# qq456cvb/VoteNet

Measured on AMD Instinct MI355X. Metric: SUN RGB-D 20k-pt scenes/sec (fwd+bwd), higher is better.
Workload: dtype f32

## Files before the change

### votenet_amd/csrc/mlp_wgrad_fast.hip

```cpp
#include "mlp_types.h"

namespace votenet {

constexpr int WF_BR = 16;

typedef short tr_v4s __attribute__((ext_vector_type(4)));
typedef __attribute__((address_space(3))) tr_v4s *tr_lds_ptr;
__device__ __forceinline__ uint4 tr_fragment(unsigned lds_off, unsigned four_rows)
{
    const tr_v4s lo = __builtin_amdgcn_ds_read_tr16_b64_v4i16((tr_lds_ptr)(uintptr_t)lds_off);
    const tr_v4s hi = __builtin_amdgcn_ds_read_tr16_b64_v4i16((tr_lds_ptr)(uintptr_t)(lds_off + four_rows));
    const uint2 a = __builtin_bit_cast(uint2, lo), b = __builtin_bit_cast(uint2, hi);
    return make_uint4(a.x, a.y, b.x, b.y);
}

template <int MODE, int TI, int TJ, int BSRC, bool BF3 = false>
__global__ __launch_bounds__(256) __attribute__((amdgpu_waves_per_eu(2, 3))) void mlp_wgrad_fast_kernel(
    MlpIn in, long rows, int cin, int cout, const float *__restrict__ dz, BnSrc bs, float *__restrict__ dw, long rows_per_block)
{
    if (bs.nh_dev != nullptr) {
        const long lim = (long)bs.nh_dev[0] * kPiece;
        rows = lim < rows ? lim : rows;
    }
    constexpr int BI = 64 * TI, BJ = 64 * TJ;
    constexpr int QA = BI / 4, QB = BJ / 4;
    constexpr int NA = WF_BR * QA / 256, NB = WF_BR * QB / 256;
    constexpr int RA = 256 / QA, RB = 256 / QB;
    __shared__ float As[BF3 ? 1 : 2][BF3 ? 1 : WF_BR][BI + 4];
    __shared__ float Bs[BF3 ? 1 : 2][BF3 ? 1 : WF_BR][BJ + 4];
    constexpr int PA = BI * 2 + 64, PB = BJ * 2 + 64;
    __shared__ __attribute__((aligned(16))) unsigned char A3[BF3 ? 2 * 3 * WF_BR * PA : 16];
    __shared__ __attribute__((aligned(16))) unsigned char B3[BF3 ? 2 * 3 * WF_BR * PB : 16];
    const int tid = threadIdx.x, lane = tid & 63;
    const int wv = __builtin_amdgcn_readfirstlane(tid >> 6);
    const int wi = wv >> 1, wj = wv & 1;
    const int i0 = blockIdx.y * BI, j0 = blockIdx.z * BJ;
    const long r_begin = (long)blockIdx.x * rows_per_block;
    if (r_begin >= rows) return;
    const int nrow = (int)((r_begin + rows_per_block < rows ? r_begin + rows_per_block : rows) - r_begin);
    const int nslab = (nrow + WF_BR - 1) / WF_BR;
    const int a_row = tid / QA, a_q = tid % QA;
    const int b_row = tid / QB, b_q = tid % QB;
    const int ka = i0 + a_q * 4;
    const int nb = j0 + b_q * 4;
    const int xc = (MODE == 0) ? cin : in.c;

    const bool affine = (MODE == 0 || MODE == 2 || MODE == 3) && in.in_scale != nullptr;
    float4 wx0 = make_float4(0.f, 0.f, 0.f, 0.f), wx1 = wx0, wx2 = wx0;
    if (MODE == 3) {
        wx0 = *reinterpret_cast<const float4 *>(in.wx + ka);
        wx1 = *reinterpret_cast<const float4 *>(in.wx + cin + ka);
        wx2 = *reinterpret_cast<const float4 *>(in.wx + 2 * cin + ka);
    }
    float w0r[4][8], b0r[4];
    if (MODE == 2) {
#pragma unroll
        for (int d = 0; d < 8; d++) {
            const float4 w4 = d < in.k0 ? *reinterpret_cast<const float4 *>(in.w0 + (size_t)d * cin + ka) : make_float4(0.f, 0.f, 0.f, 0.f);
            w0r[0][d] = w4.x;
            w0r[1][d] = w4.y;
            w0r[2][d] = w4.z;
            w0r[3][d] = w4.w;
        }
        const float4 b4 = in.b0 ? *reinterpret_cast<const float4 *>(in.b0 + ka) : make_float4(0.f, 0.f, 0.f, 0.f);
        b0r[0] = b4.x;
        b0r[1] = b4.y;
        b0r[2] = b4.z;
        b0r[3] = b4.w;
    }
    float4 csc = make_float4(1.f, 1.f, 1.f, 1.f), csh = make_float4(0.f, 0.f, 0.f, 0.f);
    if (affine) {
        csc = *reinterpret_cast<const float4 *>(in.in_scale + ka);
        csh = *reinterpret_cast<const float4 *>(in.in_shift + ka);
    }
    const float x_floor = (affine && in.in_relu) ? 0.0f : -__builtin_inff();
    float4 kA, kB, kC, kS, kH;
    kA = kB = kC = kS = kH = make_float4(0.f, 0.f, 0.f, 0.f);
    if (BSRC == 1 || BSRC == 2 || BSRC == 4) {
        kA = *reinterpret_cast<const float4 *>(bs.coef + nb);
        kB = *reinterpret_cast<const float4 *>(bs.coef + cout + nb);
        kC = *reinterpret_cast<const float4 *>(bs.coef + 2 * cout + nb);
        kS = *reinterpret_cast<const float4 *>(bs.coef + 3 * cout + nb);
        kH = *reinterpret_cast<const float4 *>(bs.coef + 4 * cout + nb);
    }
    if (BSRC == 3) {
        kS = *reinterpret_cast<const float4 *>(bs.coef + nb);
        kH = *reinterpret_cast<const float4 *>(bs.coef + cout + nb);
    }
    const float b_floor = (BSRC == 3 && bs.relu) ? 0.0f : -__builtin_inff();
    const float *xb = (MODE == 0) ? in.x + (size_t)r_begin * cin + ka : (MODE == 2) ? in.u8 + (size_t)r_begin * 8 : (MODE == 3) ? in.ptab + ka : in.feat + ka;
    const float4 *geob = (MODE == 3) ? reinterpret_cast<const float4 *>(in.geo) + r_begin : nullptr;
    const float *zb = (BSRC == 0 ? dz : bs.z) + (size_t)r_begin * cout + nb;
    const float *gb = (BSRC == 1 || BSRC == 4) ? bs.da + (size_t)r_begin * cout + nb : nullptr;
    const int *idxb = (MODE == 1) ? in.idx + r_begin : nullptr;
    const unsigned grows = (MODE == 1) ? (unsigned)in.m * (unsigned)in.nsample : 1u;

    struct Regs {
        float4 a[NA], b[NB], g[NB];
        float4 a2[(MODE == 2 || MODE == 3) ? NA : 1];
        int4 m[NB];
        float mu[NB];
        int s;
    };
    Regs R[2];
    struct Pix {
        int i;
        float4 g;
    };
    Pix pidx[NA];
    auto clampr = [&](int lr) { return lr < nrow ? lr : nrow - 1; };
    auto load_idx = [&](int s) {
        if (MODE == 1 || MODE == 3) {
#pragma unroll
            for (int h = 0; h < NA; h++) {
                const int lr = clampr(s * WF_BR + a_row + h * RA);
                if (MODE == 1) pidx[h].i = idxb[lr];
                else pidx[h].g = geob[lr];
            }
        }
    };
    auto load_slab = [&](Regs &r, int s, const Pix (&pi)[NA]) {
        r.s = s;
#pragma unroll
        for (int h = 0; h < NA; h++) {
            const int lr = clampr(s * WF_BR + a_row + h * RA);
            if (MODE == 0) {
                r.a[h] = *reinterpret_cast<const float4 *>(xb + (size_t)((unsigned)lr * (unsigned)cin));
            } else if (MODE == 2) {
                r.a[h] = *reinterpret_cast<const float4 *>(xb + (size_t)((unsigned)lr * 8u));
                r.a2[h] = *reinterpret_cast<const float4 *>(xb + (size_t)((unsigned)lr * 8u) + 4);
            } else if (MODE == 3) {
                r.a[h] = *reinterpret_cast<const float4 *>(xb + (size_t)__float_as_uint(pi[h].g.w) * cin);
                r.a2[h] = pi[h].g;
            } else {
                const unsigned scene = (unsigned)(r_begin + lr) / grows;
                r.a[h] = *reinterpret_cast<const float4 *>(xb + ((size_t)scene * in.n + pi[h].i) * xc);
            }
        }
#pragma unroll
        for (int h = 0; h < NB; h++) {
            const int lr = clampr(s * WF_BR + b_row + h * RB);
            const unsigned off = (unsigned)lr * (unsigned)cout;
            r.b[h] = *reinterpret_cast<const float4 *>(zb + (size_t)off);
            if (BSRC == 1 || BSRC == 4) r.g[h] = *reinterpret_cast<const float4 *>(gb + (size_t)off);
            if (BSRC == 4) {
                const unsigned gr = (unsigned)(r_begin + lr);
                r.mu[h] = (gr % (unsigned)kPiece) == 0u ? bs.wh[gr / (unsigned)kPiece] : 1.0f;
            }
            if (BSRC == 2) {
                const unsigned gr = (unsigned)(r_begin + lr);
                const unsigned grp = bs.pool_shift >= 0 ? gr >> bs.pool_shift : gr / (unsigned)bs.pool_k;
                r.g[h] = *reinterpret_cast<const float4 *>(bs.gout + (size_t)grp * cout + nb);
                r.m[h] = *reinterpret_cast<const int4 *>(bs.argmax + (size_t)grp * cout + nb);
            }
        }
    };
    auto store_slab = [&](int buf, const Regs &r) {
#pragma unroll
        for (int h = 0; h < NA; h++) {
            float4 v = r.a[h];
            if (MODE == 2) {
                const float4 v2 = r.a2[h];
                const float uu[8] = {v.x, v.y, v.z, v.w, v2.x, v2.y, v2.z, v2.w};
                const f32x2 z01 = narrow_z2(uu, w0r[0], w0r[1], b0r[0], b0r[1]), z23 = narrow_z2(uu, w0r[2], w0r[3], b0r[2], b0r[3]);
                v.x = z01.x;
                v.y = z01.y;
                v.z = z23.x;
                v.w = z23.y;
            }
            if (MODE == 3) {
                const float4 g = r.a2[h];
                const f32x2 z01 = assembled_z2(v.x, v.y, g, wx0.x, wx0.y, wx1.x, wx1.y, wx2.x, wx2.y);
                const f32x2 z23 = assembled_z2(v.z, v.w, g, wx0.z, wx0.w, wx1.z, wx1.w, wx2.z, wx2.w);
                v.x = z01.x;
                v.y = z01.y;
                v.z = z23.x;
                v.w = z23.y;
            }
            v.x = fmaxf(v.x * csc.x + csh.x, x_floor);
            v.y = fmaxf(v.y * csc.y + csh.y, x_floor);
            v.z = fmaxf(v.z * csc.z + csh.z, x_floor);
            v.w = fmaxf(v.w * csc.w + csh.w, x_floor);
            if constexpr (BF3) {
                unsigned h0, m0, l0, h1, m1, l1;
                split3(v.x, v.y, h0, m0, l0);
                split3(v.z, v.w, h1, m1, l1);
                unsigned char *d = A3 + ((size_t)(buf * 3) * WF_BR + a_row + h * RA) * PA + a_q * 8;
                *reinterpret_cast<uint2 *>(d) = make_uint2(h0, h1);
                *reinterpret_cast<uint2 *>(d + WF_BR * PA) = make_uint2(m0, m1);
                *reinterpret_cast<uint2 *>(d + 2 * WF_BR * PA) = make_uint2(l0, l1);
            } else {
                *reinterpret_cast<float4 *>(&As[buf][a_row + h * RA][a_q * 4]) = v;
            }
// ... 83 lines not shown
    const int nslab2 = (nslab + 1) & ~1;
    for (int s = 0; s < nslab2; s += 2) {
#pragma unroll
        for (int par = 0; par < 2; par++) {
            Regs &rs = R[par ^ 1];
            if constexpr (BF3) {
                const unsigned g = (unsigned)lane >> 4, sl = (unsigned)lane & 15u;
                const unsigned la = ((g >> 1) * 8u + (sl >> 2)) * PA + ((g & 1u) * 16u + (sl & 3u) * 4u) * 2u + (unsigned)(wi * TI) * 64u;
                const unsigned lb = ((g >> 1) * 8u + (sl >> 2)) * PB + ((g & 1u) * 16u + (sl & 3u) * 4u) * 2u + (unsigned)(wj * TJ) * 64u;
                const unsigned a0 = (unsigned)(uintptr_t)A3 + (unsigned)buf * (3u * WF_BR * PA) + la;
                const unsigned b0 = (unsigned)(uintptr_t)B3 + (unsigned)buf * (3u * WF_BR * PB) + lb;
                uint4 fa3[3][TI], fb3[3][TJ];
#pragma unroll
                for (int pc = 0; pc < 3; pc++) {
#pragma unroll
                    for (int t = 0; t < TI; t++) fa3[pc][t] = tr_fragment(a0 + (unsigned)pc * (WF_BR * PA) + (unsigned)t * 64u, 4u * PA);
#pragma unroll
                    for (int t = 0; t < TJ; t++) fb3[pc][t] = tr_fragment(b0 + (unsigned)pc * (WF_BR * PB) + (unsigned)t * 64u, 4u * PB);
                }
                auto mm = [&](int pa, int pb) {
#pragma unroll
                    for (int a = 0; a < TI; a++)
#pragma unroll
                        for (int b = 0; b < TJ; b++)
                            acc[a][b] = __builtin_amdgcn_mfma_f32_32x32x16_bf16(__builtin_bit_cast(bf16x8, fa3[pa][a]),
                                                                                __builtin_bit_cast(bf16x8, fb3[pb][b]), acc[a][b], 0, 0, 0);
                };
#ifdef WG_ABL_HALF
                mm(2, 0);
#else
                mm(2, 0);
                mm(0, 2);
                mm(1, 1);
#endif
                store_slab(buf ^ 1, rs);
#pragma unroll
                for (int h = 0; h < NA; h++) pcur[h] = pidx[h];
                load_idx(s + par + 4);
                load_slab(rs, s + par + 3, pcur);
#ifdef WG_ABL_HALF
                mm(0, 1);
                mm(0, 0);
#else
                mm(1, 0);
                mm(0, 1);
                mm(0, 0);
#endif
                lds_barrier();
                buf ^= 1;
                continue;
            }
            float fa[2][TI], fb[2][TJ];
#pragma unroll
            for (int t = 0; t < TI; t++) fa[0][t] = As[buf][kh][(wi * TI + t) * 32 + l31];
#pragma unroll
            for (int t = 0; t < TJ; t++) fb[0][t] = Bs[buf][kh][(wj * TJ + t) * 32 + l31];
#pragma unroll
            for (int k2 = 0; k2 < WF_BR / 2; k2++) {
                if (k2 == WF_BR / 4) {
                    store_slab(buf ^ 1, rs);
#pragma unroll
                    for (int h = 0; h < NA; h++) pcur[h] = pidx[h];
                    load_idx(s + par + 4);
                    load_slab(rs, s + par + 3, pcur);
                }
                if (k2 + 1 < WF_BR / 2) {
#pragma unroll
                    for (int t = 0; t < TI; t++) fa[(k2 + 1) & 1][t] = As[buf][(k2 + 1) * 2 + kh][(wi * TI + t) * 32 + l31];
#pragma unroll
                    for (int t = 0; t < TJ; t++) fb[(k2 + 1) & 1][t] = Bs[buf][(k2 + 1) * 2 + kh][(wj * TJ + t) * 32 + l31];
                }
                __builtin_amdgcn_sched_barrier(0);
#pragma unroll
                for (int a = 0; a < TI; a++)
#pragma unroll
                    for (int b = 0; b < TJ; b++)
                        acc[a][b] = __builtin_amdgcn_mfma_f32_32x32x2f32(fa[k2 & 1][a], fb[k2 & 1][b], acc[a][b], 0, 0, 0);
                __builtin_amdgcn_sched_barrier(0);
            }
            lds_barrier();
            buf ^= 1;
        }
    }
    const int wrow0 = (MODE == 1) ? 3 : 0;
#pragma unroll
    for (int a = 0; a < TI; a++)
#pragma unroll
        for (int b = 0; b < TJ; b++) {
            const int j = j0 + (wj * TJ + b) * 32 + l31;
#pragma unroll
            for (int e = 0; e < 16; e++) {
                const int i = i0 + (wi * TI + a) * 32 + (e & 3) + 8 * (e >> 2) + 4 * kh;
                const size_t off = (size_t)(wrow0 + i) * cout + j;
                if (bs.part) bs.part[(size_t)blockIdx.x * bs.pstride + off] = acc[a][b][e];
                else unsafeAtomicAdd(&dw[off], acc[a][b][e]);
            }
        }
}

int g_wgrad_fast_wgs = 0;
int g_wgrad_bf3 = 1;
static void plan_fast(long rows, int cin, int cout, int &TIr, int &TJr, int &ti, int &tj, long &rpb, unsigned &gx, bool partials)
{
    TIr = cin % 128 == 0 ? 2 : 1;
    TJr = cout % 128 == 0 ? 2 : 1;
    ti = cin / (64 * TIr);
    tj = cout / (64 * TJr);
    const int wgs = g_wgrad_fast_wgs > 0 ? g_wgrad_fast_wgs : (partials ? 256 : 384);
    long splits = wgs / (ti * tj);
    if (splits < 1) splits = 1;
    rpb = (rows + splits - 1) / splits;
    rpb = (rpb + 2 * WF_BR - 1) / (2 * WF_BR) * (2 * WF_BR);
    if (rpb < 8 * WF_BR) rpb = 8 * WF_BR;
    gx = (unsigned)((rows + rpb - 1) / rpb);
}

long wgrad_fast_slices(long rows, int cin, int cout)
{
    if (cin % 64 != 0 || cout % 64 != 0 || rows <= 0) return 0;
    int TIr, TJr, ti, tj;
    long rpb;
    unsigned gx;
    plan_fast(rows, cin, cout, TIr, TJr, ti, tj, rpb, gx, false);
    return gx;
}

void wgrad_reduce(int nslice, long pstride, long e0, long e1, const float *part, float *dw, hipStream_t st);

template <int MODE, int BSRC>
static bool launch(const MlpIn &d, long rows, int cin, int cout, const float *dz, BnSrc bs, float *dw, hipStream_t st, float *scratch)
{
    int TIr, TJr, ti, tj;
    long rpb;
    unsigned gx;
    plan_fast(rows, cin, cout, TIr, TJr, ti, tj, rpb, gx, scratch != nullptr);
    const int wide = cin > cout ? cin : cout;
    if (rpb * wide >= (1L << 31)) return false;
    const int wrow0 = (MODE == 1) ? 3 : 0;
    bs.part = scratch;
    bs.pstride = (long)(wrow0 + cin) * cout;
    const dim3 grid(gx, ti, tj);
    if (g_wgrad_bf3 && BSRC != 3) {
        if (TIr == 2 && TJr == 2)
            hipLaunchKernelGGL((mlp_wgrad_fast_kernel<MODE, 2, 2, BSRC, true>), grid, dim3(256), 0, st, d, rows, cin, cout, dz, bs, dw, rpb);
        else if (TIr == 2)
            hipLaunchKernelGGL((mlp_wgrad_fast_kernel<MODE, 2, 1, BSRC, true>), grid, dim3(256), 0, st, d, rows, cin, cout, dz, bs, dw, rpb);
        else if (TJr == 2)
            hipLaunchKernelGGL((mlp_wgrad_fast_kernel<MODE, 1, 2, BSRC, true>), grid, dim3(256), 0, st, d, rows, cin, cout, dz, bs, dw, rpb);
        else
            hipLaunchKernelGGL((mlp_wgrad_fast_kernel<MODE, 1, 1, BSRC, true>), grid, dim3(256), 0, st, d, rows, cin, cout, dz, bs, dw, rpb);
    } else if (TIr == 2 && TJr == 2)
        hipLaunchKernelGGL((mlp_wgrad_fast_kernel<MODE, 2, 2, BSRC>), grid, dim3(256), 0, st, d, rows, cin, cout, dz, bs, dw, rpb);
    else if (TIr == 2)
        hipLaunchKernelGGL((mlp_wgrad_fast_kernel<MODE, 2, 1, BSRC>), grid, dim3(256), 0, st, d, rows, cin, cout, dz, bs, dw, rpb);
    else if (TJr == 2)
        hipLaunchKernelGGL((mlp_wgrad_fast_kernel<MODE, 1, 2, BSRC>), grid, dim3(256), 0, st, d, rows, cin, cout, dz, bs, dw, rpb);
    else
        hipLaunchKernelGGL((mlp_wgrad_fast_kernel<MODE, 1, 1, BSRC>), grid, dim3(256), 0, st, d, rows, cin, cout, dz, bs, dw, rpb);
    if (scratch) wgrad_reduce((int)gx, bs.pstride, (long)wrow0 * cout, (long)(wrow0 + cin) * cout, scratch, dw, st);
    return true;
}

bool wgrad_fast_launch(int mode, const MlpIn &d, long rows, int cin, int cout, const float *dz, const BnSrc &bs, int bsrc, float *dw,
                       hipStream_t st, float *scratch)
{
    if (cin % 64 != 0 || cout % 64 != 0 || rows <= 0 || rows >= (1L << 31)) return false;
    auto al = [](const void *p) { return ((uintptr_t)p % 16) == 0; };
    if (!al(dw) || (bsrc == 0 && !al(dz)) || (bsrc != 0 && (!al(bs.z) || !al(bs.coef))) || ((bsrc == 1 || bsrc == 4) && !al(bs.da)) ||
        (bsrc == 2 && (!al(bs.gout) || !al(bs.argmax))))
        return false;
    if (mode == 0) {
        if (!al(d.x) || (d.in_scale && (!al(d.in_scale) || !al(d.in_shift)))) return false;
        if (bsrc == 0) return launch<0, 0>(d, rows, cin, cout, dz, bs, dw, st, scratch);
        if (bsrc == 1) return launch<0, 1>(d, rows, cin, cout, dz, bs, dw, st, scratch);
        if (bsrc == 3) return launch<0, 3>(d, rows, cin, cout, dz, bs, dw, st, scratch);
        return launch<0, 2>(d, rows, cin, cout, dz, bs, dw, st, scratch);
    }
    if (mode == 3) {
        if (!al(d.geo) || !al(d.ptab) || !al(d.wx) || (bsrc != 1 && bsrc != 4)) return false;
        if (d.in_scale && (!al(d.in_scale) || !al(d.in_shift))) return false;
        if (bsrc == 4) return bs.wh != nullptr && rows % 32 == 0 && launch<3, 4>(d, rows, cin, cout, dz, bs, dw, st, scratch);
        return launch<3, 1>(d, rows, cin, cout, dz, bs, dw, st, scratch);
    }
    if (mode == 2) {
        if (!al(d.u8) || !al(d.w0) || (d.b0 && !al(d.b0)) || d.k0 < 1 || d.k0 > 8 || (bsrc != 1 && bsrc != 4)) return false;
        if (d.in_scale && (!al(d.in_scale) || !al(d.in_shift))) return false;
        if (bsrc == 4) return bs.wh != nullptr && rows % 32 == 0 && launch<2, 4>(d, rows, cin, cout, dz, bs, dw, st, scratch);
        return launch<2, 1>(d, rows, cin, cout, dz, bs, dw, st, scratch);
    }
    if (d.c != cin || !al(d.feat) || bsrc != 0) return false;
    return launch<1, 0>(d, rows, cin, cout, dz, bs, dw, st, scratch);
}

}

extern "C" void votenet_debug_wgrad_workgroups(int n) { VN_DEBUG_GATE(); votenet::g_wgrad_fast_wgs = n > 0 ? n : 0; }
extern "C" void votenet_debug_wgrad_bf3(int on) { VN_DEBUG_GATE(); votenet::g_wgrad_bf3 = on ? 1 : 0; }
```

### votenet_amd/csrc/pool_bwd.hip

```cpp
#include "mlp_types.h"
#include <mutex>
#include <set>

namespace votenet {

bool wgrad_fast_launch(int mode, const MlpIn &d, long rows, int cin, int cout, const float *dz, const BnSrc &bs, int bsrc, float *dw,
                       hipStream_t st, float *scratch);
void wgrad_reduce(int nslice, long pstride, long e0, long e1, const float *part, float *dw, hipStream_t st);

static inline int pb_grid(long total, int block, int cap)
{
    long g = (total + block - 1) / block;
    if (g > cap) g = cap;
    return (int)(g < 1 ? 1 : g);
}

__global__ __launch_bounds__(256) void bn_bwd_reduce_zsel_kernel(long groups, int c, const float *__restrict__ gout,
                                                                 const float *__restrict__ zsel, const float *__restrict__ scale,
                                                                 const float *__restrict__ shift, const float *__restrict__ mean,
                                                                 const float *__restrict__ var, float eps, int relu,
                                                                 double *__restrict__ sums, CoefTail tail)
{
    __shared__ float sh1[4][64], sh2[4][64];
    const int cx = threadIdx.x & 63, ry = threadIdx.x >> 6;
// ... 958 lines not shown
                                     below_var, eps, below_relu, below_sums, below_tail, hc, wh, G, stream, nh_dev);
}

static int pool_dgrad_scatter_launch(long groups, int k, int cin, int cout, const float *gout, const int *argmax, const float *zsel,
                                     const float *coef, int relu, const float *wT, float *da, const float *below_z,
                                     const float *below_scale, const float *below_shift, const float *below_mean, const float *below_var,
                                     float eps, int below_relu, double *below_sums, const votenet_coef_tail *below_tail, const int *hc,
                                     const float *wh, int G, void *stream, const int *nh_dev)
{
    hipStream_t st = as_stream(stream);
    const PoolBelow pb = {below_z, below_scale, below_shift, below_mean, below_var, eps, below_relu, below_sums, to_tail(below_tail), g_scatter_reverse, hc, wh, G, nh_dev};
    auto go = [&](auto kern, int ci, int co, int threads = 512) {
        const size_t smem = ((size_t)co * ci + 4 * co + 4 * k) * 4;
        const int per_cu = smem > 80 * 1024 ? 1 : (smem > 40 * 1024 ? 2 : 4);
        static std::set<const void *> raised;
        static std::mutex raised_mu;
        bool fresh;
        {
            std::lock_guard<std::mutex> lock(raised_mu);
            fresh = raised.insert(reinterpret_cast<const void *>(kern)).second;
        }
        if (fresh)
            (void)hipFuncSetAttribute(reinterpret_cast<const void *>(kern), hipFuncAttributeMaxDynamicSharedMemorySize, (int)smem);
        hipLaunchKernelGGL(kern, dim3(pb_grid(groups, 2, 256 * per_cu)), dim3(threads), smem, st, groups, gout, argmax, zsel, coef, relu,
                           wT, da, pb);
    };
    auto gow = [&](auto kern, int ci, int co, int kk, int nwv) {
        const size_t smem = (size_t)co * ci * 4 + (size_t)nwv * ((co + 3 * kk) * 6 + kk * 4);
        const int per_cu = smem > 80 * 1024 ? 1 : (smem > 40 * 1024 ? 2 : 4);
        static std::set<const void *> raised_w;
        static std::mutex raised_w_mu;
        bool fresh;
        {
            std::lock_guard<std::mutex> lock(raised_w_mu);
            fresh = raised_w.insert(reinterpret_cast<const void *>(kern)).second;
        }
        if (fresh)
            (void)hipFuncSetAttribute(reinterpret_cast<const void *>(kern), hipFuncAttributeMaxDynamicSharedMemorySize, (int)smem);
        hipLaunchKernelGGL(kern, dim3(pb_grid(groups, nwv, g_scatter_wgs > 0 ? g_scatter_wgs : 256 * per_cu)), dim3(nwv * 64), smem, st, groups, gout,
                           argmax, zsel, coef, relu, wT, da, pb);
    };
    if (g_scatter_form == 1 || hc) {
#define VN_SCATTER_WAVE(CI, CO, KK, NW)                                                            \
    do {                                                                                           \
        if (below_z) gow(pool_dgrad_scatter_wave_kernel<CI, CO, KK, true, NW>, CI, CO, KK, NW);   \
        else gow(pool_dgrad_scatter_wave_kernel<CI, CO, KK, false, NW>, CI, CO, KK, NW);          \
    } while (0)
        if (hc) {
            if (cin == 64) VN_SCATTER_WAVE(64, 128, kPiece, 8);
            else if (cout == 256) {
                if (g_scatter_nwv == 12) VN_SCATTER_WAVE(128, 256, kPiece, 12);
                else VN_SCATTER_WAVE(128, 256, kPiece, 16);
            }
            else VN_SCATTER_WAVE(128, 128, kPiece, 8);
        } else {
            if (cin == 64) VN_SCATTER_WAVE(64, 128, 64, 8);
            else if (cout == 256) VN_SCATTER_WAVE(128, 256, 64, 8);
            else VN_SCATTER_WAVE(128, 128, 64, 8);
        }
#undef VN_SCATTER_WAVE
        return check_launch("pool_dgrad_scatter");
    }
    if (below_z) {
        if (cin == 128 && cout == 256)
            go(pool_dgrad_scatter_kernel<128, 256, 64, true, 16>, 128, 256, 1024);
        else if (cin == 128)
            go(pool_dgrad_scatter_kernel<128, 128, 64, true>, 128, 128);
        else
            go(pool_dgrad_scatter_kernel<64, 128, 64, true>, 64, 128);
    } else {
        if (cin == 128 && cout == 256)
            go(pool_dgrad_scatter_kernel<128, 256, 64, false, 16>, 128, 256, 1024);
        else if (cin == 128)
            go(pool_dgrad_scatter_kernel<128, 128, 64, false>, 128, 128);
        else
            go(pool_dgrad_scatter_kernel<64, 128, 64, false>, 64, 128);
    }
    return check_launch("pool_dgrad_scatter");
}

#ifndef GRAM_ABL
#define GRAM_ABL 0
#endif
template <int C, int NP = 3>
__global__ __launch_bounds__(256) void gram_bf3_kernel(long rows, const float *__restrict__ x, const float *__restrict__ scale_shift,
                                                       int relu, float *__restrict__ gram, long rows_per_block,
                                                       const float *__restrict__ wh ,
                                                       const int *__restrict__ nh_dev )
{
    if (nh_dev != nullptr) {
        const long lim = (long)nh_dev[0] * kPiece;
        rows = lim < rows ? lim : rows;
    }
    constexpr int KPT = C / 16;
    constexpr int T = C / 64;
    constexpr int PL = C * 4 + 16;
    static_assert(NP == 2 || NP == 3, "pieces per operand");
    constexpr float kA = NP == 2 ? 16.0f : 1.0f, kUn = NP == 2 ? 1.0f / 256.0f : 1.0f;
    __shared__ __attribute__((aligned(16))) unsigned Ts[2][NP][2][PL];
    const int tid = threadIdx.x, lane = tid & 63;
    const int wv = __builtin_amdgcn_readfirstlane(tid >> 6);
    const int wi = wv >> 1, wj = wv & 1;
    const long r_begin = (long)blockIdx.x * rows_per_block;
    if (r_begin >= rows) return;
    const int nrow = (int)((r_begin + rows_per_block < rows ? r_begin + rows_per_block : rows) - r_begin);
    const int nslab = (nrow + 15) / 16;
    const int c = tid % C, rg = tid / C;
    const int kh_w = (C == 128) ? rg : (rg >> 1), d_w = (C == 128) ? 0 : (rg & 1) * 2;
    const float sc = scale_shift[c] * kA, sh = scale_shift[C + c] * kA;
    const float floor_ = relu ? 0.0f : -__builtin_inff();
    const float *xb = x + (size_t)r_begin * C + c;
    float R[2][KPT];
    static_assert(kPiece == 16, "one slab = one piece");
    const bool first_rg = rg == 0;
    const float *whb = wh ? wh + r_begin / kPiece : nullptr;
    const float *whp = whb ? whb : scale_shift;
    float Wq[2] = {1.0f, 1.0f};
    bool abl_prologue = true;
    auto load = [&](float (&r)[KPT], int s, float &wq) {
        if ((GRAM_ABL & 4) && !abl_prologue) return;
#pragma unroll
        for (int i = 0; i < KPT; i++) {
            int lr = s * 16 + rg * KPT + i;
            lr = lr < nrow ? lr : nrow - 1;
            r[i] = xb[(size_t)lr * C];
        }
        const int sw = (whb != nullptr && s * 16 < nrow) ? s : 0;
        wq = whp[sw];
    };
    auto store = [&](int buf, const float (&r)[KPT], int s, float wq) {
        if ((GRAM_ABL & 8) && !abl_prologue) return;
        float v[KPT];
#pragma unroll
        for (int i = 0; i < KPT; i++) {
            v[i] = fmaxf(r[i] * sc + sh, floor_);
            if (s * 16 + rg * KPT + i >= nrow) v[i] = 0.0f;
        }
        if (whb != nullptr && first_rg && s * 16 < nrow) v[0] *= sqrtf(wq);
        if constexpr (NP == 2) {
            unsigned h[KPT / 2], l[KPT / 2];
#pragma unroll
            for (int i = 0; i < KPT / 2; i++) split2(v[2 * i], v[2 * i + 1], h[i], l[i]);
            if constexpr (C == 128) {
                *reinterpret_cast<uint4 *>(&Ts[buf][0][kh_w][c * 4]) = make_uint4(h[0], h[1], h[2], h[3]);
                *reinterpret_cast<uint4 *>(&Ts[buf][1][kh_w][c * 4]) = make_uint4(l[0], l[1], l[2], l[3]);
            } else {
                *reinterpret_cast<uint2 *>(&Ts[buf][0][kh_w][c * 4 + d_w]) = make_uint2(h[0], h[1]);
                *reinterpret_cast<uint2 *>(&Ts[buf][1][kh_w][c * 4 + d_w]) = make_uint2(l[0], l[1]);
            }
            return;
        }
        unsigned h[KPT / 2], m[KPT / 2], l[KPT / 2];
#pragma unroll
        for (int i = 0; i < KPT / 2; i++) split3(v[2 * i], v[2 * i + 1], h[i], m[i], l[i]);
        if constexpr (C == 128) {
            *reinterpret_cast<uint4 *>(&Ts[buf][0][kh_w][c * 4]) = make_uint4(h[0], h[1], h[2], h[3]);
            *reinterpret_cast<uint4 *>(&Ts[buf][1][kh_w][c * 4]) = make_uint4(m[0], m[1], m[2], m[3]);
            *reinterpret_cast<uint4 *>(&Ts[buf][NP - 1][kh_w][c * 4]) = make_uint4(l[0], l[1], l[2], l[3]);
        } else {
            *reinterpret_cast<uint2 *>(&Ts[buf][0][kh_w][c * 4 + d_w]) = make_uint2(h[0], h[1]);
            *reinterpret_cast<uint2 *>(&Ts[buf][1][kh_w][c * 4 + d_w]) = make_uint2(m[0], m[1]);
            *reinterpret_cast<uint2 *>(&Ts[buf][NP - 1][kh_w][c * 4 + d_w]) = make_uint2(l[0], l[1]);
        }
    };
    f32x16 acc[T][T];
#pragma unroll
    for (int a = 0; a < T; a++)
#pragma unroll
        for (int b = 0; b < T; b++)
#pragma unroll
            for (int e = 0; e < 16; e++) acc[a][b][e] = 0.0f;
    load(R[0], 0, Wq[0]);
    store(0, R[0], 0, Wq[0]);
    load(R[1], 1, Wq[1]);
    __builtin_amdgcn_sched_barrier(0);
    load(R[0], 2, Wq[0]);
    __syncthreads();
    const int kh = lane >> 5, l31 = lane & 31;
    int buf = 0;
    abl_prologue = false;
    const int nslab2 = (nslab + 1) & ~1;
    for (int s = 0; s < nslab2; s += 2) {
#pragma unroll
        for (int par = 0; par < 2; par++) {
            uint4 fa[NP][T], fb[NP][T];
#pragma unroll
            for (int p = 0; p < NP; p++) {
#pragma unroll
                for (int t = 0; t < T; t++) {
                    fa[p][t] = *reinterpret_cast<const uint4 *>(&Ts[buf][p][kh][((wi * T + t) * 32 + l31) * 4]);
                    fb[p][t] = *reinterpret_cast<const uint4 *>(&Ts[buf][p][kh][((wj * T + t) * 32 + l31) * 4]);
                }
            }
            auto mm = [&](int pa, int pb) {
                if (GRAM_ABL & 1) {
                    acc[0][0][0] += __uint_as_float(fa[pa][0].x ^ fb[pb][0].y);
                    return;
                }
#pragma unroll
                for (int a = 0; a < T; a++)
#pragma unroll
                    for (int b = 0; b < T; b++) {
                        if constexpr (NP == 2)
                            acc[a][b] = __builtin_amdgcn_mfma_f32_32x32x16_f16(__builtin_bit_cast(f16x8, fa[pa][a]),
                                                                               __builtin_bit_cast(f16x8, fb[pb][b]), acc[a][b], 0, 0, 0);
                        else
                            acc[a][b] = __builtin_amdgcn_mfma_f32_32x32x16_bf16(__builtin_bit_cast(bf16x8, fa[pa][a]),
                                                                                __builtin_bit_cast(bf16x8, fb[pb][b]), acc[a][b], 0, 0, 0);
                    }
            };
            if constexpr (NP == 2) {
                mm(1, 0);
                mm(0, 1);
                store(buf ^ 1, R[par ^ 1], s + par + 1, Wq[par ^ 1]);
                load(R[par ^ 1], s + par + 3, Wq[par ^ 1]);
                mm(0, 0);
            } else {
                mm(2, 0);
                mm(0, 2);
                mm(1, 1);
                store(buf ^ 1, R[par ^ 1], s + par + 1, Wq[par ^ 1]);
                load(R[par ^ 1], s + par + 3, Wq[par ^ 1]);
                mm(1, 0);
                mm(0, 1);
                mm(0, 0);
            }
            lds_barrier();
            buf ^= 1;
        }
    }
    if (GRAM_ABL & 2) {
        float t_ = 0.0f;
#pragma unroll
        for (int a = 0; a < T; a++)
#pragma unroll
            for (int b = 0; b < T; b++)
#pragma unroll
                for (int e = 0; e < 16; e++) t_ += acc[a][b][e];
        if (t_ == 12345.678f) gram[0] = t_;
        return;
    }
#pragma unroll
    for (int a = 0; a < T; a++)
#pragma unroll
        for (int b = 0; b < T; b++) {
            const int j = (wj * T + b) * 32 + l31;
#pragma unroll
            for (int e = 0; e < 16; e++) {
                const int i = (wi * T + a) * 32 + (e & 3) + 8 * (e >> 2) + 4 * kh;
                unsafeAtomicAdd(&gram[(size_t)i * C + j], acc[a][b][e] * kUn);
            }
        }
}

int g_gram_bf3 = 1;
static int g_gram_wgs = 384;
template <int C>
static void gram_bf3_launch(long rows, const float *z, const float *scale_shift, int relu, float *gram, hipStream_t st, const float *wh = nullptr,
                            const int *nh_dev = nullptr)
{
    long rpb = (rows + g_gram_wgs - 1) / g_gram_wgs;
    rpb = (rpb + 31) / 32 * 32;
    if (rpb < 128) rpb = 128;
    const unsigned gx = (unsigned)((rows + rpb - 1) / rpb);
    if (g_gram_bf3 != 3) hipLaunchKernelGGL((gram_bf3_kernel<C, 2>), dim3(gx), dim3(256), 0, st, rows, z, scale_shift, relu, gram, rpb, wh, nh_dev);
    else hipLaunchKernelGGL((gram_bf3_kernel<C, 3>), dim3(gx), dim3(256), 0, st, rows, z, scale_shift, relu, gram, rpb, wh, nh_dev);
}
extern "C" void votenet_debug_gram_bf3(int on) { VN_DEBUG_GATE(); g_gram_bf3 = on; }
extern "C" void votenet_debug_gram_workgroups(int n) { VN_DEBUG_GATE(); g_gram_wgs = n > 0 ? n : 384; }

extern "C" int votenet_mlp_gram(long rows, int c, const float *z, const float *scale_shift, int relu, float *gram, float *scratch,
                                void *stream)
{
    if (g_gram_bf3 && scratch == nullptr && (c == 64 || c == 128) && rows > 0 && rows < (1L << 31) / c && z && scale_shift && gram &&
        (uintptr_t)z % 16 == 0) {
        if (c == 128) gram_bf3_launch<128>(rows, z, scale_shift, relu, gram, as_stream(stream));
        else gram_bf3_launch<64>(rows, z, scale_shift, relu, gram, as_stream(stream));
        return check_launch("mlp_gram");
    }
    VN_REQUIRE(rows > 0 && c > 0 && z && scale_shift && gram, "mlp_gram: bad arguments");
    MlpIn d = {};
    d.x = z;
    d.in_scale = scale_shift;
    d.in_shift = scale_shift + c;
    d.in_relu = relu;
    BnSrc bs = {};
    bs.z = z;
    bs.coef = scale_shift;
    bs.relu = relu;
    VN_REQUIRE(wgrad_fast_launch(0, d, rows, c, c, nullptr, bs, 3, gram, as_stream(stream), scratch),
               "mlp_gram: shape not served (c %% 64 == 0, 16-byte aligned operands), got c = %d", c);
    return check_launch("mlp_gram");
}

static int g_sparse_wgs = 384, g_sparse_wgs2 = 256, g_sparse_teams = 2;
extern "C" void votenet_debug_sparse_workgroups(int n) { VN_DEBUG_GATE(); g_sparse_wgs = n > 0 ? n : 384; }
extern "C" void votenet_debug_sparse_teams(int teams, int wgs)
{
    VN_DEBUG_GATE();
    g_sparse_teams = teams == 1 ? 1 : 2;
    if (wgs > 0) g_sparse_wgs2 = wgs;
}
static int pool_wgrad_sparse_launch(long groups, int cin, int cout, const float *xz, const float *in_scale, const float *in_shift, int in_relu,
                                    const float *gout, const int *argmax, const float *zsel, const float *coef, int relu, float *dw,
                                    float *colsum, float *scratch, const int *hc, const float *wh, int G, void *stream, const int *nh_dev = nullptr);
extern "C" int votenet_pool_wgrad_sparse(long groups, int k, int cin, int cout, const float *xz, const float *in_scale,
                                         const float *in_shift, int in_relu, const float *gout, const int *argmax, const float *zsel,
                                         const float *coef, int relu, float *dw, float *colsum, float *scratch, void *stream)
{
    VN_REQUIRE(groups > 0 && xz && gout && argmax && zsel && coef && dw && colsum, "pool_wgrad_sparse: bad arguments");
    VN_REQUIRE(cin <= cout, "pool_wgrad_sparse expects cin <= cout");
    VN_REQUIRE(votenet_pool_backward_supported(cin, cout, k), "pool_wgrad_sparse: unsupported shape cin=%d cout=%d k=%d", cin, cout, k);
    VN_REQUIRE((in_scale == nullptr) == (in_shift == nullptr), "pool_wgrad_sparse: in_scale and in_shift go together");
    VN_REQUIRE((uintptr_t)xz % 16 == 0 && (!in_scale || ((uintptr_t)in_scale % 16 == 0 && (uintptr_t)in_shift % 16 == 0)),
               "pool_wgrad_sparse: operands must be 16-byte aligned");
    return pool_wgrad_sparse_launch(groups, cin, cout, xz, in_scale, in_shift, in_relu, gout, argmax, zsel, coef, relu, dw, colsum, scratch,
                                    nullptr, nullptr, 0, stream);
}

extern "C" int votenet_mlp_gram_half(long rows, int c, const float *z, const float *scale_shift, int relu, const float *wh, float *gram,
                                     const int *nh_dev, void *stream)
{
    VN_REQUIRE(rows > 0 && rows % kPiece == 0 && rows < (1L << 31) / c && (c == 128 || c == 64), "mlp_gram_half expects rows %% 16 == 0 and c in {64, 128}");
    VN_REQUIRE(z && scale_shift && wh && gram && (uintptr_t)z % 16 == 0, "mlp_gram_half: null / unaligned buffer");
    if (c == 128) gram_bf3_launch<128>(rows, z, scale_shift, relu, gram, as_stream(stream), wh, nh_dev);
    else gram_bf3_launch<64>(rows, z, scale_shift, relu, gram, as_stream(stream), wh, nh_dev);
    return check_launch("mlp_gram_half");
}

extern "C" int votenet_pool_wgrad_sparse_half(long nh, int G, int cin, int cout, const float *xz, const float *in_scale, const float *in_shift,
                                              int in_relu, const float *gout, const int *argmax, const float *zsel, const float *coef, int relu,
                                              float *dw, float *colsum, const int *hc, const float *wh, const int *nh_dev, void *stream)
{
    VN_REQUIRE(nh > 0 && G > 0 && nh >= G && nh <= (long)kBallPieces * G && hc && wh, "pool_wgrad_sparse_half: bad piece-layout arguments");
    VN_REQUIRE(xz && gout && argmax && zsel && coef && dw && colsum, "pool_wgrad_sparse_half: bad arguments");
    VN_REQUIRE(votenet_pool_backward_supported(cin, cout, 64), "pool_wgrad_sparse_half: unsupported shape cin=%d cout=%d", cin, cout);
    VN_REQUIRE((in_scale == nullptr) == (in_shift == nullptr), "pool_wgrad_sparse_half: in_scale and in_shift go together");
    VN_REQUIRE((uintptr_t)xz % 16 == 0 && (!in_scale || ((uintptr_t)in_scale % 16 == 0 && (uintptr_t)in_shift % 16 == 0)),
               "pool_wgrad_sparse_half: operands must be 16-byte aligned");
    return pool_wgrad_sparse_launch(nh, cin, cout, xz, in_scale, in_shift, in_relu, gout, argmax, zsel, coef, relu, dw, colsum, nullptr, hc, wh,
                                    G, stream, nh_dev);
}

static int g_sparse_centre_wgs = 192, g_sparse_centre_teams = 2;
extern "C" void votenet_debug_sparse_centre_workgroups(int n) { VN_DEBUG_GATE(); g_sparse_centre_wgs = n > 0 ? n : 192; }
extern "C" void votenet_debug_sparse_centre_teams(int t) { VN_DEBUG_GATE(); g_sparse_centre_teams = t == 1 ? 1 : 2; }
extern "C" int votenet_pool_wgrad_sparse_half_centres(long nh, int G, int cin, int cout, const float *xz, const float *in_scale,
                                                      const float *in_shift, int in_relu, const float *gout, const int *argmax,
                                                      const float *zsel, const float *coef, int relu, float *dw, float *colsum,
                                                      const int *pos, const float *wh, const int *nh_dev, void *stream)
{
    VN_REQUIRE(nh > 0 && G > 0 && nh >= G && nh <= (long)kBallPieces * G && pos && wh, "pool_wgrad_sparse_half_centres: bad piece-layout arguments");
// ... 90 lines not shown
```

Baseline: 2284.

## Add multi-team workgroups to wgrad and gram kernels with in-LDS reduction

Both the weight-gradient kernel (for 128x128) and the Gram kernel now launch workgroups containing several 256-thread teams. Each team processes its own row range in its own dynamic-LDS region, and the partial accumulators are reduced through LDS before a single team issues the global atomics. This is meant to cut global atomic traffic and the number of workgroups while keeping the total wave count. The cost is much larger LDS per workgroup (the dynamic-LDS limit is raised once per kernel), extra barriers, and lower occupancy per CU.

```diff
diff --git a/votenet_amd/csrc/mlp_wgrad_fast.hip b/votenet_amd/csrc/mlp_wgrad_fast.hip
--- a/votenet_amd/csrc/mlp_wgrad_fast.hip
+++ b/votenet_amd/csrc/mlp_wgrad_fast.hip
@@ -1,4 +1,5 @@
 #include "mlp_types.h"
+#include <mutex>
 
 namespace votenet {
 
@@ -14,10 +15,12 @@
     return make_uint4(a.x, a.y, b.x, b.y);
 }
 
-template <int MODE, int TI, int TJ, int BSRC, bool BF3 = false>
-__global__ __launch_bounds__(256) __attribute__((amdgpu_waves_per_eu(2, 3))) void mlp_wgrad_fast_kernel(
+extern __shared__ __attribute__((aligned(16))) unsigned char wgrad_team_smem[];
+template <int MODE, int TI, int TJ, int BSRC, bool BF3 = false, int TEAMS = 1>
+__global__ __launch_bounds__(256 * TEAMS) __attribute__((amdgpu_waves_per_eu(2, 3))) void mlp_wgrad_fast_kernel(
     MlpIn in, long rows, int cin, int cout, const float *__restrict__ dz, BnSrc bs, float *__restrict__ dw, long rows_per_block)
 {
+    static_assert(TEAMS == 1 || (TEAMS == 2 && BF3), "teams: the split-operand form only");
     if (bs.nh_dev != nullptr) {
         const long lim = (long)bs.nh_dev[0] * kPiece;
         rows = lim < rows ? lim : rows;
@@ -29,16 +32,23 @@
     __shared__ float As[BF3 ? 1 : 2][BF3 ? 1 : WF_BR][BI + 4];
     __shared__ float Bs[BF3 ? 1 : 2][BF3 ? 1 : WF_BR][BJ + 4];
     constexpr int PA = BI * 2 + 64, PB = BJ * 2 + 64;
-    __shared__ __attribute__((aligned(16))) unsigned char A3[BF3 ? 2 * 3 * WF_BR * PA : 16];
-    __shared__ __attribute__((aligned(16))) unsigned char B3[BF3 ? 2 * 3 * WF_BR * PB : 16];
-    const int tid = threadIdx.x, lane = tid & 63;
+    __shared__ __attribute__((aligned(16))) unsigned char A3s[BF3 && TEAMS == 1 ? 2 * 3 * WF_BR * PA : 16];
+    __shared__ __attribute__((aligned(16))) unsigned char B3s[BF3 && TEAMS == 1 ? 2 * 3 * WF_BR * PB : 16];
+    const int tid = TEAMS > 1 ? (int)(threadIdx.x & 255) : (int)threadIdx.x, lane = tid & 63;
+    const int team = TEAMS > 1 ? __builtin_amdgcn_readfirstlane((int)(threadIdx.x >> 8)) : 0;
     const int wv = __builtin_amdgcn_readfirstlane(tid >> 6);
     const int wi = wv >> 1, wj = wv & 1;
+    unsigned char *const A3 = TEAMS > 1 ? wgrad_team_smem + team * (2 * 3 * WF_BR * (PA + PB)) : A3s;
+    unsigned char *const B3 = TEAMS > 1 ? A3 + 2 * 3 * WF_BR * PA : B3s;
     const int i0 = blockIdx.y * BI, j0 = blockIdx.z * BJ;
-    const long r_begin = (long)blockIdx.x * rows_per_block;
-    if (r_begin >= rows) return;
-    const int nrow = (int)((r_begin + rows_per_block < rows ? r_begin + rows_per_block : rows) - r_begin);
-    const int nslab = (nrow + WF_BR - 1) / WF_BR;
+    const long wg_begin = (long)blockIdx.x * TEAMS * rows_per_block;
+    if (wg_begin >= rows) return;
+    const long r_team = wg_begin + team * rows_per_block;
+    const int nrow = r_team >= rows ? 0 : (int)((r_team + rows_per_block < rows ? r_team + rows_per_block : rows) - r_team);
+    const long r_begin = nrow > 0 ? r_team : 0;
+    const int last = nrow > 0 ? nrow - 1 : 0;
+    const long left0 = rows - wg_begin;
+    const int nslab = (int)(((left0 < rows_per_block ? left0 : rows_per_block) + WF_BR - 1) / WF_BR);
     const int a_row = tid / QA, a_q = tid % QA;
     const int b_row = tid / QB, b_q = tid % QB;
     const int ka = i0 + a_q * 4;
@@ -108,7 +118,7 @@
         float4 g;
     };
     Pix pidx[NA];
-    auto clampr = [&](int lr) { return lr < nrow ? lr : nrow - 1; };
+    auto clampr = [&](int lr) { return lr < nrow ? lr : last; };
     auto load_idx = [&](int s) {
         if (MODE == 1 || MODE == 3) {
 #pragma unroll
@@ -358,6 +368,34 @@
             buf ^= 1;
         }
     }
+    if constexpr (TEAMS > 1) {
+        float4 *comb = reinterpret_cast<float4 *>(wgrad_team_smem) + tid;
+        if (team == 1) {
+#pragma unroll
+            for (int a = 0; a < TI; a++)
+#pragma unroll
+                for (int b = 0; b < TJ; b++)
+#pragma unroll
+                    for (int q = 0; q < 4; q++)
+                        comb[((a * TJ + b) * 4 + q) * 256] = make_float4(acc[a][b][4 * q], acc[a][b][4 * q + 1], acc[a][b][4 * q + 2], acc[a][b][4 * q + 3]);
+        }
+        lds_barrier();
+        if (team == 1) return;
+#pragma unroll
+        for (int a = 0; a < TI; a++)
+#pragma unroll
+            for (int b = 0; b < TJ; b++) {
+#pragma unroll
+                for (int q = 0; q < 4; q++) {
+                    const float4 v = comb[((a * TJ + b) * 4 + q) * 256];
+                    acc[a][b][4 * q] += v.x;
+                    acc[a][b][4 * q + 1] += v.y;
+                    acc[a][b][4 * q + 2] += v.z;
+                    acc[a][b][4 * q + 3] += v.w;
+                }
+                __builtin_amdgcn_sched_barrier(0);
+            }
+    }
     const int wrow0 = (MODE == 1) ? 3 : 0;
 #pragma unroll
     for (int a = 0; a < TI; a++)
@@ -376,19 +414,26 @@
 
 int g_wgrad_fast_wgs = 0;
 int g_wgrad_bf3 = 1;
-static void plan_fast(long rows, int cin, int cout, int &TIr, int &TJr, int &ti, int &tj, long &rpb, unsigned &gx, bool partials)
+#ifndef WGRAD_TEAMS
+#define WGRAD_TEAMS 2
+#define WGRAD_TEAM_WGS 256
+#endif
+static int g_wgrad_team_wgs = WGRAD_TEAM_WGS;
+static bool plan_teams(int cin, int cout, bool partials) { return WGRAD_TEAMS == 2 && g_wgrad_bf3 && cin == 128 && cout == 128 && !partials; }
+static void plan_fast(long rows, int cin, int cout, int &TIr, int &TJr, int &ti, int &tj, long &rpb, unsigned &gx, bool partials, int teams = 1)
 {
     TIr = cin % 128 == 0 ? 2 : 1;
     TJr = cout % 128 == 0 ? 2 : 1;
     ti = cin / (64 * TIr);
     tj = cout / (64 * TJr);
-    const int wgs = g_wgrad_fast_wgs > 0 ? g_wgrad_fast_wgs : (partials ? 256 : 384);
+    const int wgs = g_wgrad_fast_wgs > 0 ? g_wgrad_fast_wgs : (partials ? 256 : teams > 1 ? g_wgrad_team_wgs : 384);
     long splits = wgs / (ti * tj);
     if (splits < 1) splits = 1;
+    splits *= teams;
     rpb = (rows + splits - 1) / splits;
     rpb = (rpb + 2 * WF_BR - 1) / (2 * WF_BR) * (2 * WF_BR);
     if (rpb < 8 * WF_BR) rpb = 8 * WF_BR;
-    gx = (unsigned)((rows + rpb - 1) / rpb);
+    gx = (unsigned)((rows + rpb * teams - 1) / (rpb * teams));
 }
 
 long wgrad_fast_slices(long rows, int cin, int cout)
@@ -409,14 +454,24 @@
     int TIr, TJr, ti, tj;
     long rpb;
     unsigned gx;
-    plan_fast(rows, cin, cout, TIr, TJr, ti, tj, rpb, gx, scratch != nullptr);
+    const bool teams = plan_teams(cin, cout, scratch != nullptr) && BSRC != 3 && MODE != 2;
+    plan_fast(rows, cin, cout, TIr, TJr, ti, tj, rpb, gx, scratch != nullptr, teams ? 2 : 1);
     const int wide = cin > cout ? cin : cout;
     if (rpb * wide >= (1L << 31)) return false;
     const int wrow0 = (MODE == 1) ? 3 : 0;
     bs.part = scratch;
     bs.pstride = (long)(wrow0 + cin) * cout;
     const dim3 grid(gx, ti, tj);
-    if (g_wgrad_bf3 && BSRC != 3) {
+    if (teams) {
+        if constexpr (BSRC != 3 && MODE != 2 && WGRAD_TEAMS == 2) {
+            constexpr int PA = 128 * 2 + 64;
+            constexpr size_t smem = 2 * (size_t)(2 * 3 * WF_BR * (PA + PA));
+            auto kern = mlp_wgrad_fast_kernel<MODE, 2, 2, BSRC, true, 2>;
+            static std::once_flag raised;
+            std::call_once(raised, [&] { (void)hipFuncSetAttribute(reinterpret_cast<const void *>(kern), hipFuncAttributeMaxDynamicSharedMemorySize, (int)smem); });
+            hipLaunchKernelGGL(kern, grid, dim3(512), smem, st, d, rows, cin, cout, dz, bs, dw, rpb);
+        }
+    } else if (g_wgrad_bf3 && BSRC != 3) {
         if (TIr == 2 && TJr == 2)
             hipLaunchKernelGGL((mlp_wgrad_fast_kernel<MODE, 2, 2, BSRC, true>), grid, dim3(256), 0, st, d, rows, cin, cout, dz, bs, dw, rpb);
         else if (TIr == 2)
diff --git a/votenet_amd/csrc/pool_bwd.hip b/votenet_amd/csrc/pool_bwd.hip
--- a/votenet_amd/csrc/pool_bwd.hip
+++ b/votenet_amd/csrc/pool_bwd.hip
@@ -1064,11 +1064,11 @@
 #ifndef GRAM_ABL
 #define GRAM_ABL 0
 #endif
-template <int C, int NP = 3>
-__global__ __launch_bounds__(256) void gram_bf3_kernel(long rows, const float *__restrict__ x, const float *__restrict__ scale_shift,
-                                                       int relu, float *__restrict__ gram, long rows_per_block,
-                                                       const float *__restrict__ wh ,
-                                                       const int *__restrict__ nh_dev )
+template <int C, int NP = 3, int TEAMS = 1>
+__global__ __launch_bounds__(256 * TEAMS) void gram_bf3_kernel(long rows, const float *__restrict__ x, const float *__restrict__ scale_shift,
+                                                               int relu, float *__restrict__ gram, long rows_per_team,
+                                                               const float *__restrict__ wh ,
+                                                               const int *__restrict__ nh_dev )
 {
     if (nh_dev != nullptr) {
         const long lim = (long)nh_dev[0] * kPiece;
@@ -1079,23 +1079,31 @@
     constexpr int PL = C * 4 + 16;
     static_assert(NP == 2 || NP == 3, "pieces per operand");
     constexpr float kA = NP == 2 ? 16.0f : 1.0f, kUn = NP == 2 ? 1.0f / 256.0f : 1.0f;
-    __shared__ __attribute__((aligned(16))) unsigned Ts[2][NP][2][PL];
-    const int tid = threadIdx.x, lane = tid & 63;
+    extern __shared__ __attribute__((aligned(16))) unsigned gram_smem[];
+    const int tid = threadIdx.x & 255, lane = tid & 63;
+    const int team = TEAMS > 1 ? __builtin_amdgcn_readfirstlane((int)(threadIdx.x >> 8)) : 0;
     const int wv = __builtin_amdgcn_readfirstlane(tid >> 6);
     const int wi = wv >> 1, wj = wv & 1;
-    const long r_begin = (long)blockIdx.x * rows_per_block;
-    if (r_begin >= rows) return;
-    const int nrow = (int)((r_begin + rows_per_block < rows ? r_begin + rows_per_block : rows) - r_begin);
-    const int nslab = (nrow + 15) / 16;
+    unsigned *const Tteam = gram_smem + team * (2 * NP * 2 * PL);
+    auto Ts = [&](int buf, int p, int kh_) -> unsigned * { return Tteam + ((buf * NP + p) * 2 + kh_) * PL; };
+    const long wg_begin = (long)blockIdx.x * TEAMS * rows_per_team;
+    if (wg_begin >= rows) return;
+    const long left0 = rows - wg_begin;
+    const int nslab0 = (int)(((left0 < rows_per_team ? left0 : rows_per_team) + 15) / 16);
+    const long r_team = wg_begin + team * rows_per_team;
+    const long left = rows - r_team;
+    const int nrow = left <= 0 ? 0 : (int)(left < rows_per_team ? left : rows_per_team);
+    const int last = nrow > 0 ? nrow - 1 : 0;
+    const long r_begin = nrow > 0 ? r_team : 0;
     const int c = tid % C, rg = tid / C;
     const int kh_w = (C == 128) ? rg : (rg >> 1), d_w = (C == 128) ? 0 : (rg & 1) * 2;
     const float sc = scale_shift[c] * kA, sh = scale_shift[C + c] * kA;
     const float floor_ = relu ? 0.0f : -__builtin_inff();
-    const float *xb = x + (size_t)r_begin * C + c;
+    const char *xb = reinterpret_cast<const char *>(x + (size_t)r_begin * C);
     float R[2][KPT];
     static_assert(kPiece == 16, "one slab = one piece");
     const bool first_rg = rg == 0;
-    const float *whb = wh ? wh + r_begin / kPiece : nullptr;
+    const float *whb = (wh && nrow > 0) ? wh + r_begin / kPiece : nullptr;
     const float *whp = whb ? whb : scale_shift;
     float Wq[2] = {1.0f, 1.0f};
     bool abl_prologue = true;
@@ -1104,8 +1112,8 @@
 #pragma unroll
         for (int i = 0; i < KPT; i++) {
             int lr = s * 16 + rg * KPT + i;
-            lr = lr < nrow ? lr : nrow - 1;
-            r[i] = xb[(size_t)lr * C];
+            lr = lr < nrow ? lr : last;
+            r[i] = *reinterpret_cast<const float *>(xb + (unsigned)(lr * C + c) * 4u);
         }
         const int sw = (whb != nullptr && s * 16 < nrow) ? s : 0;
         wq = whp[sw];
@@ -1124,11 +1132,11 @@
 #pragma unroll
             for (int i = 0; i < KPT / 2; i++) split2(v[2 * i], v[2 * i + 1], h[i], l[i]);
             if constexpr (C == 128) {
-                *reinterpret_cast<uint4 *>(&Ts[buf][0][kh_w][c * 4]) = make_uint4(h[0], h[1], h[2], h[3]);
-                *reinterpret_cast<uint4 *>(&Ts[buf][1][kh_w][c * 4]) = make_uint4(l[0], l[1], l[2], l[3]);
+                *reinterpret_cast<uint4 *>(Ts(buf, 0, kh_w) + c * 4) = make_uint4(h[0], h[1], h[2], h[3]);
+                *reinterpret_cast<uint4 *>(Ts(buf, 1, kh_w) + c * 4) = make_uint4(l[0], l[1], l[2], l[3]);
             } else {
-                *reinterpret_cast<uint2 *>(&Ts[buf][0][kh_w][c * 4 + d_w]) = make_uint2(h[0], h[1]);
-                *reinterpret_cast<uint2 *>(&Ts[buf][1][kh_w][c * 4 + d_w]) = make_uint2(l[0], l[1]);
+                *reinterpret_cast<uint2 *>(Ts(buf, 0, kh_w) + c * 4 + d_w) = make_uint2(h[0], h[1]);
+                *reinterpret_cast<uint2 *>(Ts(buf, 1, kh_w) + c * 4 + d_w) = make_uint2(l[0], l[1]);
             }
             return;
         }
@@ -1136,13 +1144,13 @@
 #pragma unroll
         for (int i = 0; i < KPT / 2; i++) split3(v[2 * i], v[2 * i + 1], h[i], m[i], l[i]);
         if constexpr (C == 128) {
-            *reinterpret_cast<uint4 *>(&Ts[buf][0][kh_w][c * 4]) = make_uint4(h[0], h[1], h[2], h[3]);
-            *reinterpret_cast<uint4 *>(&Ts[buf][1][kh_w][c * 4]) = make_uint4(m[0], m[1], m[2], m[3]);
-            *reinterpret_cast<uint4 *>(&Ts[buf][NP - 1][kh_w][c * 4]) = make_uint4(l[0], l[1], l[2], l[3]);
+            *reinterpret_cast<uint4 *>(Ts(buf, 0, kh_w) + c * 4) = make_uint4(h[0], h[1], h[2], h[3]);
+            *reinterpret_cast<uint4 *>(Ts(buf, 1, kh_w) + c * 4) = make_uint4(m[0], m[1], m[2], m[3]);
+            *reinterpret_cast<uint4 *>(Ts(buf, NP - 1, kh_w) + c * 4) = make_uint4(l[0], l[1], l[2], l[3]);
         } else {
-            *reinterpret_cast<uint2 *>(&Ts[buf][0][kh_w][c * 4 + d_w]) = make_uint2(h[0], h[1]);
-            *reinterpret_cast<uint2 *>(&Ts[buf][1][kh_w][c * 4 + d_w]) = make_uint2(m[0], m[1]);
-            *reinterpret_cast<uint2 *>(&Ts[buf][NP - 1][kh_w][c * 4 + d_w]) = make_uint2(l[0], l[1]);
+            *reinterpret_cast<uint2 *>(Ts(buf, 0, kh_w) + c * 4 + d_w) = make_uint2(h[0], h[1]);
+            *reinterpret_cast<uint2 *>(Ts(buf, 1, kh_w) + c * 4 + d_w) = make_uint2(m[0], m[1]);
+            *reinterpret_cast<uint2 *>(Ts(buf, NP - 1, kh_w) + c * 4 + d_w) = make_uint2(l[0], l[1]);
         }
     };
     f32x16 acc[T][T];
@@ -1161,7 +1169,7 @@
     const int kh = lane >> 5, l31 = lane & 31;
     int buf = 0;
     abl_prologue = false;
-    const int nslab2 = (nslab + 1) & ~1;
+    const int nslab2 = (nslab0 + 1) & ~1;
     for (int s = 0; s < nslab2; s += 2) {
 #pragma unroll
         for (int par = 0; par < 2; par++) {
@@ -1170,8 +1178,8 @@
             for (int p = 0; p < NP; p++) {
 #pragma unroll
                 for (int t = 0; t < T; t++) {
-                    fa[p][t] = *reinterpret_cast<const uint4 *>(&Ts[buf][p][kh][((wi * T + t) * 32 + l31) * 4]);
-                    fb[p][t] = *reinterpret_cast<const uint4 *>(&Ts[buf][p][kh][((wj * T + t) * 32 + l31) * 4]);
+                    fa[p][t] = *reinterpret_cast<const uint4 *>(Ts(buf, p, kh) + ((wi * T + t) * 32 + l31) * 4);
+                    fb[p][t] = *reinterpret_cast<const uint4 *>(Ts(buf, p, kh) + ((wj * T + t) * 32 + l31) * 4);
                 }
             }
             auto mm = [&](int pa, int pb) {
@@ -1222,6 +1230,40 @@
         if (t_ == 12345.678f) gram[0] = t_;
         return;
     }
+    if constexpr (TEAMS > 1) {
+        float4 *comb = reinterpret_cast<float4 *>(gram_smem) + tid;
+        for (int t = 1; t < TEAMS; t++) {
+            if (team == t) {
+#pragma unroll
+                for (int a = 0; a < T; a++)
+#pragma unroll
+                    for (int b = 0; b < T; b++)
+#pragma unroll
+                        for (int q = 0; q < 4; q++)
+                            comb[((a * T + b) * 4 + q) * 256] =
+                                make_float4(acc[a][b][4 * q], acc[a][b][4 * q + 1], acc[a][b][4 * q + 2], acc[a][b][4 * q + 3]);
+            }
+            lds_barrier();
+            if (team == 0) {
+#pragma unroll
+                for (int a = 0; a < T; a++)
+#pragma unroll
+                    for (int b = 0; b < T; b++) {
+#pragma unroll
+                        for (int q = 0; q < 4; q++) {
+                            const float4 v = comb[((a * T + b) * 4 + q) * 256];
+                            acc[a][b][4 * q] += v.x;
+                            acc[a][b][4 * q + 1] += v.y;
+                            acc[a][b][4 * q + 2] += v.z;
+                            acc[a][b][4 * q + 3] += v.w;
+                        }
+                        __builtin_amdgcn_sched_barrier(0);
+                    }
+            }
+            if (t + 1 < TEAMS) lds_barrier();
+        }
+        if (team != 0) return;
+    }
 #pragma unroll
     for (int a = 0; a < T; a++)
 #pragma unroll
@@ -1236,20 +1278,42 @@
 }
 
 int g_gram_bf3 = 1;
-static int g_gram_wgs = 384;
+#ifndef GRAM_TEAMS_128
+#define GRAM_TEAMS_128 4
+#define GRAM_TEAMS_64 4
+#define GRAM_WGS 192
+#endif
+static int g_gram_wgs = GRAM_WGS;
+template <int C, int NP, int TEAMS>
+static void gram_bf3_go(long rows, const float *z, const float *scale_shift, int relu, float *gram, hipStream_t st, const float *wh, const int *nh_dev)
+{
+    const long shares = (long)g_gram_wgs * TEAMS;
+    long rpt = (rows + shares - 1) / shares;
+    rpt = (rpt + 31) / 32 * 32;
+    if (rpt < 128) rpt = 128;
+    const long cap = ((1L << 30) / C - 1) / 32 * 32;
+    if (rpt > cap) rpt = cap;
+    const unsigned gx = (unsigned)((rows + rpt * TEAMS - 1) / (rpt * TEAMS));
+    constexpr size_t image = (size_t)TEAMS * 2 * NP * 2 * (C * 4 + 16) * 4, tile = TEAMS > 1 ? (size_t)C * C * 4 : 0;
+    constexpr size_t smem = image > tile ? image : tile;
+    auto kern = gram_bf3_kernel<C, NP, TEAMS>;
+    if (smem > 64 * 1024) {
+        static std::once_flag raised;
+        std::call_once(raised, [&] { (void)hipFuncSetAttribute(reinterpret_cast<const void *>(kern), hipFuncAttributeMaxDynamicSharedMemorySize, (int)smem); });
+    }
+    hipLaunchKernelGGL(kern, dim3(gx), dim3(256 * TEAMS), smem, st, rows, z, scale_shift, relu, gram, rpt, wh, nh_dev);
+}
 template <int C>
 static void gram_bf3_launch(long rows, const float *z, const float *scale_shift, int relu, float *gram, hipStream_t st, const float *wh = nullptr,
                             const int *nh_dev = nullptr)
 {
-    long rpb = (rows + g_gram_wgs - 1) / g_gram_wgs;
-    rpb = (rpb + 31) / 32 * 32;
-    if (rpb < 128) rpb = 128;
-    const unsigned gx = (unsigned)((rows + rpb - 1) / rpb);
-    if (g_gram_bf3 != 3) hipLaunchKernelGGL((gram_bf3_kernel<C, 2>), dim3(gx), dim3(256), 0, st, rows, z, scale_shift, relu, gram, rpb, wh, nh_dev);
-    else hipLaunchKernelGGL((gram_bf3_kernel<C, 3>), dim3(gx), dim3(256), 0, st, rows, z, scale_shift, relu, gram, rpb, wh, nh_dev);
+    constexpr int TEAMS = C == 128 ? GRAM_TEAMS_128 : GRAM_TEAMS_64;
+    constexpr int TEAMS3 = (C == 128 && TEAMS > 2) ? 2 : TEAMS;
+    if (g_gram_bf3 != 3) gram_bf3_go<C, 2, TEAMS>(rows, z, scale_shift, relu, gram, st, wh, nh_dev);
+    else gram_bf3_go<C, 3, TEAMS3>(rows, z, scale_shift, relu, gram, st, wh, nh_dev);
 }
 extern "C" void votenet_debug_gram_bf3(int on) { VN_DEBUG_GATE(); g_gram_bf3 = on; }
-extern "C" void votenet_debug_gram_workgroups(int n) { VN_DEBUG_GATE(); g_gram_wgs = n > 0 ? n : 384; }
+extern "C" void votenet_debug_gram_workgroups(int n) { VN_DEBUG_GATE(); g_gram_wgs = n > 0 ? n : GRAM_WGS; }
 
 extern "C" int votenet_mlp_gram(long rows, int c, const float *z, const float *scale_shift, int relu, float *gram, float *scratch,
                                 void *stream)
```

Measured after the change: 2276. About the same (-0.4%).
